# CILAB-MA/gpudrive_lab

Hardware: AMD Instinct MI355X
Metric: agent-steps/sec at 1024 worlds x 64 agents; achieved HBM GB/s on obs kernel (higher is better)
Workload: dtype f32

## Files before the change

### gpudrive_lab_amd/csrc/engine.cpp

```cpp
#include <hip/hip_runtime.h>

#include <algorithm>
#include <cmath>
#include <cstdlib>
#include <cstdio>
#include <cstring>
#include <map>
#include <memory>
#include <stdexcept>
#include <atomic>
#include <exception>
#include <string>
#include <thread>
#include <vector>

#include "dev_mem.hpp"
#include "engine.hpp"
#include "gd_math.hpp"
#include "scene.hpp"
#ifdef GD_CLOCKS
namespace gd { void set_clocks_read(unsigned long long *out); void step_clocks_read(unsigned long long *out); }
#endif
#ifndef GD_GRID_MIN_CELL
#define GD_GRID_MIN_CELL 16.f
// ... 155 lines not shown
    int64_t host_skipped = 0;
    bool rk_possible = false;
    bool rk_alloc = false;

    bool ensure_rank_buffers() {
        if (rk_alloc) return true;
        const size_t WA = static_cast<size_t>(W) * A;
        std::vector<gd::DevMem> mine;
        gd::DevSim n = d;
        try {
            alloc_into(mine, n.rk_E, WA * GD_RANK_CAP + 64);
            alloc_into(mine, n.rk_spc, WA * GD_RANK_SPL);
            if (std::getenv("GPUDRIVE_RANK_ALLOC_FAIL") != nullptr)
                throw HipError("GPUDRIVE_RANK_ALLOC_FAIL: simulated allocation failure of the rank replay's buffers");
            alloc_into(mine, n.rk_kt, WA * GD_RANK_KT);
            alloc_into(mine, n.rk_heap, WA * GD_RANK_HEAP_DW);
            alloc_into(mine, n.rk_cpe, WA * GD_RANK_NCP);
            alloc_into(mine, n.rk_n, WA);
            alloc_into(mine, n.rk_fallback, WA / 32);
            alloc_into(mine, n.rk_streak, WA / 32);
            alloc_into(mine, n.cp_road, 2 * WA * GD_RANK_NCP);
            alloc_into(mine, n.cp_T, 2 * WA * GD_RANK_NCP);
            alloc_into(mine, n.cp_hdr, 2 * WA);
            alloc_into(mine, n.rk_cp, WA * GD_RANK_NCP);
            alloc_into(mine, n.rk_tl, WA);
            alloc_into(mine, n.rk_hist, GD_RH_ALLOC);
            alloc_into(mine, n.rk_ticket, WA);
            alloc_into(mine, n.rk_order, WA);
            alloc_into(mine, n.rk_list, 8 * WA);
            n.rk_nlong = static_cast<int>(std::max<size_t>(WA / 4, 64));
            alloc_into(mine, n.rk_longlist, n.rk_nlong);
            alloc_into(mine, n.rk_longslot, WA);
            alloc_into(mine, n.rk_E_long, static_cast<size_t>(n.rk_nlong) * GD_RANK_CAP_LONG + 64);
            alloc_into(mine, n.rk_kt_long, static_cast<size_t>(n.rk_nlong) * GD_RANK_KT_LONG);
            internal.reserve(internal.size() + mine.size());
        } catch (const HipError &) {
            (void)hipGetLastError();
            rk_possible = false;
            d.rk_on = 0;
            return false;
        }
        for (gd::DevMem &m : mine) internal.push_back(std::move(m));
        d = n;
        rk_alloc = true;
        return true;
    }
    bool timing = false;
    std::vector<EventPair> ev_pool[gd::KERNEL_TIMED];
// ... 798 lines not shown
        s->lin_cap = (static_cast<size_t>(W) + 64) * static_cast<size_t>(A) + 8 * 4 * static_cast<size_t>(d.lin_apw) + 64;
        s->d_lin_list = s->alloc_internal<int32_t>(s->lin_cap);
        s->d_lin_list_dyn = s->alloc_internal<int32_t>(s->lin_cap);
        d.lin_list = s->d_lin_list; d.lin_list_dyn = s->d_lin_list_dyn;
        d.lin_blocks = 0; d.lin_blocks_dyn = 0; d.lin_dyn_off = 0;
        d.lin_on = std::getenv("GPUDRIVE_LINEAR_LEGACY") == nullptr ? 1 : 0;
        d.pose_stamp = s->alloc_internal<uint4>(WA);
        d.pose_skip = std::getenv("GPUDRIVE_NO_POSE_SKIP") == nullptr ? 1 : 0;
        d.stat_skipped = s->alloc_internal<unsigned long long>(GD_SKIP_SLOTS);
        s->d_row_of_slot = s->alloc_internal<int32_t>(WA);
        s->d_slot_of_row = s->alloc_internal<int32_t>(WA);
        s->d_row_count = s->alloc_internal<int32_t>(1);
        d.bad_actions = s->alloc_internal<unsigned long long>(1);
        d.blk_off = s->d_blk_off = s->alloc_internal<int32_t>(W + 1);
        d.warm_k = 0;
        d.warm_all = 0;
        d.warm_flags = s->alloc_internal<int32_t>(W);
        d.warm_count = s->alloc_internal<unsigned long long>(1);
        d.rk_on = 0;
        d.rk_dbg = 0;
        d.rk_min_roads = 1536;
        d.rk_waves = 0;
        if (const char *e = std::getenv("GPUDRIVE_RANK_WAVES")) d.rk_waves = std::min(std::max((std::atoi(e) + 7) / 8 * 8, 8), GD_RANK_GRID);
        s->rk_possible = GD_MAP_OBS_AW == 32 && cfg->knn_order != GD_KNN_SET_ORDER &&
                         params->roadObservationAlgorithm == GD_ROADS_K_NEAREST && std::getenv("GPUDRIVE_NO_RANK_REPLAY") == nullptr;
#ifdef GD_DIAG
        if (const char *e = std::getenv("GPUDRIVE_RANK_DBG")) d.rk_dbg = std::atoi(e);
#endif
        for (int i = 0; i < gd_sim::kRing; i++) {
            void *pinned = nullptr;
            HIP_CHECK(hipHostMalloc(&pinned, sizeof(int32_t) * W, hipHostMallocDefault));
            s->h_flags[i].reset(static_cast<int32_t *>(pinned));
            s->flag_ev[i] = make_event(hipEventDisableTiming);
        }
        std::vector<int> all(W);
        for (int w = 0; w < W; w++) all[w] = w;
        s->rebuild_worlds(all);
        s->do_reset(std::vector<int32_t>(W, 1));
        HIP_CHECK(hipStreamSynchronize(s->stream));
    });
    if (rc != GD_OK) return rc;
    *out = s.release();
    return GD_OK;
}

void gd_destroy(gd_sim *sim) { delete sim; }
// ... 1259 lines not shown
            return fail(GD_ERR_DEVICE, "gd_stat: reading the LiDAR flags failed");
        int64_t c = 0;
        for (int w = 0; w < s->W; w++)
            for (int a = 0; a < n[static_cast<size_t>(w) * 2] && a < s->A; a++) c += f[static_cast<size_t>(w) * s->A + a] != 0;
        *out = c;
        return GD_OK;
    }
    if (s && out && which == 45) {
        unsigned long long v = 0;
        (void)hipStreamSynchronize(s->stream);
        if (hipMemcpy(&v, s->d.bad_actions, sizeof(v), hipMemcpyDeviceToHost) != hipSuccess)
            return fail(GD_ERR_DEVICE, "gd_stat: reading the action counter failed");
        *out = static_cast<int64_t>(v);
        return GD_OK;
    }
    if (s && out && which == 46) {
        unsigned long long v = 0;
        (void)hipStreamSynchronize(s->stream);
        if (hipMemcpy(&v, s->d.warm_count, sizeof(v), hipMemcpyDeviceToHost) != hipSuccess)
            return fail(GD_ERR_DEVICE, "gd_stat: reading the warm-up counter failed");
        *out = static_cast<int64_t>(v);
        return GD_OK;
    }
    if (s && out && which == 21) {
        *out = 0;
        if (s->rk_alloc) {
            int32_t v = 0;
            (void)hipStreamSynchronize(s->stream);
            if (hipMemcpy(&v, s->d.rk_hist + GD_RANK_AUDIT, sizeof(v), hipMemcpyDeviceToHost) != hipSuccess)
                return fail(GD_ERR_DEVICE, "gd_stat: reading the audit counter failed");
            *out = v;
        }
        return GD_OK;
    }
    if (!s || !out || which < 0 || which > kLastStat) return fail(GD_ERR_INVALID, "gd_stat: bad argument");
#if defined(GD_DIAG) || defined(GD_CLOCKS)
    if (which >= 8) {
        *out = 0;
        if (s->rk_alloc) {
            int32_t v = 0;
            (void)hipStreamSynchronize(s->stream);
            (void)hipMemcpy(&v, s->d.rk_hist + 514 + (which - 8), sizeof(v), hipMemcpyDeviceToHost);
            (void)hipMemset(s->d.rk_hist + 514 + (which - 8), 0, sizeof(v));
            *out = v;
        }
        return GD_OK;
// ... 157 lines not shown
```

### gpudrive_lab_amd/csrc/engine.hpp

```cpp
#pragma once
#include <hip/hip_runtime.h>

#include <cstdint>

#include "../../include/gpudrive_amd.h"

#ifndef GD_MAP_OBS_AW
#define GD_MAP_OBS_AW 32
#endif

#define GD_RANK_CAP 1280
#define GD_RANK_NCP 40
#define GD_RANK_HEAP_DW 104
#define GD_RANK_CAP_LONG 2560
#define GD_RANK_KT_LONG 164
#define GD_RH_LONG 537
#define GD_RH_CURSOR 544
#define GD_RH_CURSOR_STRIDE 32
#define GD_RH_SIZE (GD_RH_CURSOR + 8 * GD_RH_CURSOR_STRIDE)
#define GD_RANK_GRID (256 * 8 * 4)
#ifdef GD_CLOCKS
#define GD_WAVE_CLOCKS
#endif
#ifdef GD_WAVE_CLOCKS
#define GD_RH_WAVES GD_RH_SIZE
#define GD_RH_ALLOC (GD_RH_WAVES + 3 * GD_RANK_GRID)
#else
#define GD_RH_ALLOC GD_RH_SIZE
#endif
#define GD_RANK_NCH 320
#define GD_RANK_SPL 256
#define GD_RANK_KT 84
#define GD_RANK_AUDIT 536
#define GD_LIN_BLK 16
#define GD_SKIP_SLOTS 4096

#ifdef GD_DIAG
#define GD_DIAG_IS(field, value) ((field) == (value))
#else
#define GD_DIAG_IS(field, value) false
#endif

namespace gd {

enum { KERNEL_STATE = 0, KERNEL_MAP_OBS = 1, KERNEL_LIDAR = 2, KERNEL_BEV = 3, KERNEL_PARTNER = 4, KERNEL_RESET = 5, KERNEL_PADDING = 6, KERNEL_TIMED = 5 };

struct GridHdr {
    float ox, oy, inv_cell;
    int nx, ny;
    int cell_base;
    int item_base;
    int pad;
// ... 65 lines not shown
    unsigned long long *bad_actions;
    unsigned long long *stat_skipped;
    int split_partner;
    int step_dbg;
    int rk_on;
    int rk_max_roads;
    int rk_min_roads;
    int rk_dbg;
    uint16_t *rk_E;
    int rk_nlong;
    int32_t *rk_longlist;
    int32_t *rk_longslot;
    uint16_t *rk_E_long;
    float *rk_kt_long;
    uint16_t *rk_spc;
    float *rk_kt;
    uint32_t *rk_heap;
    uint16_t *rk_cpe;
    int32_t *rk_hist;
    int rk_waves;
    int32_t *rk_ticket;
    int32_t *rk_order;
    int32_t *rk_list;
    uint2 *rk_cp;
    float *rk_tl;
    const float4 *road_bbox;
    const float *road_rbmax;
    int32_t *rk_n;
    int32_t *rk_fallback;
    int32_t *rk_streak;
    uint16_t *cp_road;
    float *cp_T;
    float4 *cp_hdr;
    int warm_k;
    int warm_all;
    int32_t *warm_flags;
    unsigned long long *warm_count;
    const float *pack_weights;
};

void launch_kernel(const DevSim &d, hipStream_t st, int which, bool move);
void launch_map_obs(const DevSim &d, hipStream_t st, bool move);
void launch_map_obs_rank(const DevSim &d, hipStream_t st);
void launch_map_obs_linear(const DevSim &d, hipStream_t st, bool move);
void launch_bev(const DevSim &d, hipStream_t st);
void launch_lidar(const DevSim &d, hipStream_t st);
void launch_pack_obs(const DevSim &d, hipStream_t st, float *out);
void launch_expert_actions(const DevSim &d, hipStream_t st, float *actions, float *pos, float *vel, float *yaw, int *valid);
void launch_set_log_actions(const DevSim &d, hipStream_t st, int t);
void launch_episode_step(const DevSim &d, hipStream_t st, const gd_episode_config &c, const gd_episode_buffers &b);
void launch_draw_weights(const DevSim &d, hipStream_t st, const gd_episode_config &c, const gd_episode_buffers &b,
                         const int32_t *worlds, int n);
void launch_pack_obs_rows(const DevSim &d, hipStream_t st, float *out,
                          const float *weights);
void launch_learner_rows(hipStream_t st, const uint8_t *mask, size_t slots, int32_t *row_of_slot, int32_t *slot_of_row,
                         int32_t *count);
void launch_discrete_actions(const DevSim &d, hipStream_t st, const int64_t *indices, const float *table, int n_actions);
void launch_pack_obs_conditioned(const DevSim &d, hipStream_t st, const float *weights, float *out);
void launch_record(const DevSim &d, hipStream_t st, const gd_record_buffers &b, int t, bool pre);
void launch_bc_rollout_row(const DevSim &d, hipStream_t st, const gd_bc_rollout_buffers &b, int t, int num_stack);
void launch_bc_rollout_actions(const DevSim &d, hipStream_t st, const gd_bc_rollout_buffers &b, int t);
void launch_bc_rollout_post(const DevSim &d, hipStream_t st, const gd_bc_rollout_buffers &b, int t, bool more);
void launch_bc_rollout_summary(hipStream_t st, const gd_bc_rollout_buffers &b);
void launch_policy_rollout_actions(const DevSim &d, hipStream_t st, const gd_policy_rollout_buffers &b, int t);
void launch_policy_rollout_book(const DevSim &d, hipStream_t st, const gd_policy_rollout_buffers &b, int t);
void launch_policy_rollout_finish(const DevSim &d, hipStream_t st, const gd_policy_rollout_buffers &b, int n_steps);
// ... 69 lines not shown
```

### gpudrive_lab_amd/csrc/map_obs_rank.hip

```cpp
#include <hip/hip_runtime.h>

#include <algorithm>
#include <type_traits>

#include "engine.hpp"
#include "gd_math.hpp"
#include "rank_cand.hpp"
#include "rank_heap.hpp"

namespace gd {

namespace {

constexpr int K = GD_MAP_OBS_K;
constexpr int CAP = GD_RANK_CAP;
constexpr int NCP = GD_RANK_NCP;
constexpr int SPL = GD_RANK_SPL;
constexpr int KT = GD_RANK_KT;
constexpr int TILE = 32;
constexpr int CAP_LONG = GD_RANK_CAP_LONG;
template <int CAP_T>
struct RankGeo {
    static constexpr bool LONG = CAP_T > CAP;
    static constexpr int NG = CAP_T / 64;
// ... 77 lines not shown
}
__device__ __forceinline__ uint2 stream_load(const uint2 *p) {
    const u2v v = __builtin_nontemporal_load(reinterpret_cast<const u2v *>(p));
    return make_uint2(v.x, v.y);
}
__device__ __forceinline__ void stream_store(uint2 v, uint2 *p) {
    u2v t; t.x = v.x; t.y = v.y;
    __builtin_nontemporal_store(t, reinterpret_cast<u2v *>(p));
}

__device__ __forceinline__ int audited(const DevSim &d, int idx, int size) {
    if ((unsigned int)idx < (unsigned int)size) return idx;
    atomicAdd(&d.rk_hist[GD_RANK_AUDIT], 1);
    return idx < 0 ? 0 : size - 1;
}

__device__ __forceinline__ bool rank_lt(unsigned int a, unsigned int b, unsigned int tm = 31u) { return (a | tm) < b; }

template <int A_T>
__global__ __launch_bounds__(256) void k_knn_scan(DevSim d) {
    if (d.gate_any && *d.any_reset == 0) return;
    constexpr int HALVES = A_T / 64;
    const int w = blockIdx.x / HALVES, a0 = (blockIdx.x % HALVES) * 64;
    const int tid = threadIdx.x, wave = tid >> 6, lane = tid & 63;
    const int n = d.shape[w * 2 + 0];
    if (a0 >= n) return;
    const int a = a0 + lane;
    const bool live = a < n;
    const size_t i = (size_t)w * A_T + a;
    const size_t WA = (size_t)d.W * A_T;
    const int r0 = d.road_off[w];
    const int R = d.road_off[w + 1] - r0;

    __shared__ unsigned short s_first[NCP][64];
    __shared__ float s_thr[NCP][64];
    __shared__ int s_ncp[64];
    __shared__ unsigned int s_needy[2];
    __shared__ float4 s_hdr[64];
    __shared__ float s_bx[64], s_by[64], s_bm[64];
    __shared__ unsigned int s_hist[4][256];

    float ex = 0.f, ey = 0.f;
    if (live) { ex = d.px[i]; ey = d.py[i]; }
    unsigned long long ranked = 0ull;
    int list_base = 0;
    if (wave == 0) {
        int ncp = 0;
        float4 h0 = make_float4(0.f, 0.f, __int_as_float(0), 0.f), h1 = h0;
        if (live) { h0 = d.cp_hdr[i]; h1 = d.cp_hdr[WA + i]; }
        s_hdr[lane] = h0;
        wave_sync();
        if (live) {
            const float4 bb = d.road_bbox[w];
            const float ddx = fmaxf(fmaxf(bb.x - ex, ex - bb.z), 0.f), ddy = fmaxf(fmaxf(bb.y - ey, ey - bb.w), 0.f);
            const float far = d.p.observationRadius * 1.01f + 1.f;
            int state = 1, reason = -1;
            if (R >= K && ddx * ddx + ddy * ddy > far * far) {
                state = RK_FAR;
                d.sel_hdr[i * 2] = make_float4(ex, ey, d.qw[i], d.qz[i]);
                d.sel_hdr[i * 2 + 1] = make_float4(__int_as_float(0), __int_as_float(r0), 0.f, 0.f);
                d.cp_hdr[i] = make_float4(ex, ey, __int_as_float(0), 0.f);
            } else {
                const int n0 = __float_as_int(h0.z), n1 = __float_as_int(h1.z);
                const float m0 = n0 > 0 ? sqrtf((ex - h0.x) * (ex - h0.x) + (ey - h0.y) * (ey - h0.y)) : __builtin_inff();
                const float m1 = n1 > 0 ? sqrtf((ex - h1.x) * (ex - h1.x) + (ey - h1.y) * (ey - h1.y)) : __builtin_inff();
                int set = m1 < m0 ? 1 : 0;
                float move = set ? m1 : m0;
                int n_cp = set ? n1 : n0;
                size_t src = i;
                if (move > 6.f) {
                    float best = move;
                    int donor = -1;
                    for (int j = 0; j < 64; j++) {
                        const float4 hj = s_hdr[j];
                        const float dj = __float_as_int(hj.z) > 0 ? sqrtf((ex - hj.x) * (ex - hj.x) + (ey - hj.y) * (ey - hj.y)) : __builtin_inff();
                        if (dj < best) { best = dj; donor = j; }
                    }
                    if (donor >= 0) {
                        move = best;
                        set = 0;
                        n_cp = __float_as_int(s_hdr[donor].z);
                        src = (size_t)w * A_T + a0 + donor;
                    }
                }
                const bool eligible = R >= K && R >= d.rk_min_roads && R <= d.rk_max_roads;
                const int grp = (int)(i / 32);
                const bool bypass = eligible && d.rk_streak[grp] >= 3 && ((d.rk_hist[513] + grp) & 63) != 0;
                const float iw = d.qw[i], iz = d.qz[i];
                const float z2 = iz * iz;
                const float det = (1.f - 2.f * z2) * (1.f - 2.f * z2) + 4.f * z2 * (iw * iw);
                const float margin = 1.00001f / fminf(det, 1.f);
                if (!eligible || bypass) {
                    state = 0;
                    ncp = 0;
                    reason = bypass ? -5 : -2;
                    d.rk_fallback[i / 32] = 1;
                } else if (n_cp <= 0 || move > 6.f) {
                    ncp = -1;
                    s_bx[lane] = ex; s_by[lane] = ey; s_bm[lane] = margin;
                } else {
                    ncp = n_cp;
                    const unsigned short *cr = d.cp_road + ((size_t)set * WA + src) * NCP;
                    const float *ct = d.cp_T + ((size_t)set * WA + src) * NCP;
                    float t = 1.f;
                    unsigned int fmax = 0u;
                    for (int q = 0; q < ncp; q++) {
                        t = ct[q];
                        const float reach = sqrtf(t) * 1.0001f + move * 1.0001f + 1e-3f;
                        float thr = reach * reach * 1.0001f * margin;
                        if (!(thr >= 0.f)) thr = __builtin_inff();
                        fmax = rank_cand::running_max(fmax, cr[q]);
                        s_first[q][lane] = (unsigned short)fmax;
                        s_thr[q][lane] = thr;
                    }
                    d.rk_tl[i] = t;
                }
            }
            d.rk_n[i] = state;
            d.rk_ticket[i] = reason;
            if (state == RK_FAR) ncp = 0;
        }
        s_ncp[lane] = ncp;
        {
            const unsigned long long nd = __ballot(ncp < 0);
            if (lane == 0) { s_needy[0] = (unsigned int)nd; s_needy[1] = (unsigned int)(nd >> 32); }
        }
        if (ncp < 0) ncp = 1;
        ranked = __ballot(ncp > 0);
        if (ranked != 0ull && lane == 0) list_base = atomicAdd(&d.rk_hist[528 + (blockIdx.x & 7)], __popcll(ranked));
    }
    __syncthreads();
    {
        const unsigned long long needy = (unsigned long long)s_needy[0] | (unsigned long long)s_needy[1] << 32;
        if (needy != 0ull) {
            constexpr int BASE = (127 - 2) << 4;
            unsigned int *hist = s_hist[wave];
            int turn = 0;
            for (unsigned long long rest = needy; rest != 0ull; rest &= rest - 1ull, turn++) {
                if ((turn & 3) != wave) continue;
                const int al = __ffsll((long long)rest) - 1;
                const float bx = s_bx[al], by = s_by[al], mg = s_bm[al];
#pragma unroll
                for (int k = 0; k < 4; k++) hist[k * 64 + lane] = 0u;
                if (lane == 0) { s_first[0][al] = (unsigned short)((K / 32) * 32); s_thr[0][al] = __builtin_inff(); }
                const float ratio = exp2f(log2f(fmaxf((float)R / 256.f, 1.f)) / (float)(NCP - 2));
                float pf = 256.f, tlast = __builtin_inff();
                int pq = 256, q = 1;
                float2 nxt = lane < R ? d.road_xy[r0 + lane] : make_float2(0.f, 0.f);
                for (int rb = 0; rb < R; rb += 64) {
                    const float2 xy = nxt;
                    if (rb + 64 + lane < R) nxt = d.road_xy[r0 + rb + 64 + lane];
                    if (rb + lane < R) {
// ... 9 lines not shown
                        int jb = 0, before = excl;
                        if (before + (int)h.x < K) { before += (int)h.x; jb = 1;
                            if (before + (int)h.y < K) { before += (int)h.y; jb = 2;
                                if (before + (int)h.z < K) { jb = 3; } } }
                        const unsigned long long cross = __ballot(excl < K && incl >= K);
                        const int Lc = __ffsll((long long)cross) - 1;
                        const int bucket = 4 * Lc + __builtin_amdgcn_readlane(jb, Lc);
                        const float T = bucket >= 255 ? __builtin_inff() : __uint_as_float((unsigned int)(bucket + 1 + BASE) << 19);
                        if (lane == 0) {
                            const float reach = sqrtf(T) * 1.0001f + 1e-3f;
                            float thr = reach * reach * 1.0001f * mg * 1.001f;
                            if (!(thr >= 0.f)) thr = __builtin_inff();
                            s_first[q][al] = (unsigned short)min(pq, 65535);
                            s_thr[q][al] = thr;
                        }
                        tlast = T;
                        q++;
                        pf *= ratio;
                        pq = max(pq + 64, ((int)pf + 63) & ~63);
                    }
                }
                if (lane == 0) {
                    s_ncp[al] = q;
                    d.rk_tl[(size_t)w * A_T + a0 + al] = tlast < 1e30f ? tlast : 1.f;
                }
            }
            __syncthreads();
        }
    }
    const int ncp = s_ncp[lane];
    if (__syncthreads_or(ncp > 0 ? 1 : 0) == 0) return;
    {
        uint2 *rows = d.rk_cp + ((size_t)w * A_T + a0) * NCP;
        for (int e = tid; e < 64 * NCP; e += 256) {
            const int ag = e / NCP, q = e - ag * NCP;
            const int n_ag = s_ncp[ag];
            if (n_ag > 0)
                rows[e] = q < n_ag ? make_uint2((unsigned int)s_first[q][ag], __float_as_uint(s_thr[q][ag]))
                                   : make_uint2(rank_cand::NO_CP, __float_as_uint(__builtin_inff()));
        }
    }
    if (wave == 0 && ranked != 0ull) {
        list_base = __builtin_amdgcn_readfirstlane(list_base);
        if (ncp > 0)
            d.rk_list[(size_t)(blockIdx.x & 7) * WA + audited(d, list_base + __popcll(ranked & ((1ull << lane) - 1ull)), (int)WA)] = (int)i;
    }
}

template <int CAP_T>
struct RankLds {
    union {
        struct {
            float ckey[CAP_T];
            unsigned short cidx[CAP_T];
        } c;
        struct {
            float skey[CAP_T];
            unsigned short spos[CAP_T];
        } s;
        unsigned short spc[CAP_T];
    };
    unsigned int cnt2[RankGeo<CAP_T>::NB / 2];
};
static_assert(sizeof(RankLds<CAP>) <= 10240 && sizeof(RankLds<CAP_LONG>) <= 20480, "sixteen / eight waves per CU");
constexpr int LSTN = (GD_MAX_ROAD_ENTITIES + GD_LIN_BLK - 1) / GD_LIN_BLK + 15;
constexpr int LSTN4 = (LSTN + 3) & ~3;
static_assert(LSTN4 <= 1024 && NCP < 64 && rank_cand::CHUNK % GD_LIN_BLK == 0 && 64 % GD_LIN_BLK == 0, "block and count share 16 bits; a block inside one chunk; whole blocks per pass");
constexpr size_t CAND_TABLES = LSTN4 * sizeof(unsigned short) + (NCP + 1) * sizeof(float);
static_assert(CAND_TABLES <= sizeof(RankLds<CAP>::cnt2) && CAND_TABLES <= sizeof(RankLds<CAP_LONG>::cnt2), "the tables fit the idle counters of both instantiations");
constexpr int CP_EPL = ((GD_MAX_ROAD_ENTITIES + rank_cand::CHUNK - 1) / rank_cand::CHUNK + 63) / 64;
static_assert(64 * CP_EPL * (sizeof(unsigned int) + sizeof(uint2)) <= sizeof(float) * CAP, "the chunk table fits the candidate keys of both instantiations");

struct RankIn {
    int i, state, r0, R, b0, li;
    float ex, ey, iw, iz, t_last;
    unsigned int cfirst;
    float cthr;
};
template <typename T>
__device__ __forceinline__ T uniform_load(const T *p) {
    return *reinterpret_cast<const __attribute__((address_space(4))) T *>(reinterpret_cast<uintptr_t>(p));
}
template <int A_T>
__device__ __forceinline__ RankIn rank_fetch(const DevSim &d, const int *list, int li, int count, int lane) {
    RankIn in;
    in.li = li;
    in.i = li < count ? uniform_load(list + li) : 0;
    in.state = li < count ? uniform_load(d.rk_n + in.i) : 0;
    const int w = in.i / A_T;
    in.r0 = uniform_load(d.road_off + w);
    in.R = uniform_load(d.road_off + w + 1) - in.r0;
    in.ex = uniform_load(d.px + in.i); in.ey = uniform_load(d.py + in.i);
    in.iw = uniform_load(d.qw + in.i); in.iz = -uniform_load(d.qz + in.i);
    in.t_last = uniform_load(d.rk_tl + in.i);
    in.b0 = uniform_load(d.blk_off + w);
    uint2 cp = make_uint2(rank_cand::NO_CP, __float_as_uint(__builtin_inff()));
    if (in.state == 1 && lane < NCP) cp = stream_load(d.rk_cp + (size_t)in.i * NCP + (unsigned int)lane);
    in.cfirst = cp.x;
    in.cthr = __uint_as_float(cp.y);
    return in;
}

#ifdef GD_CLOCKS
struct PhaseClock {
    unsigned int prev, sum[8];
    __device__ __forceinline__ void mark(int n) {
        const unsigned int t = (unsigned int)__builtin_amdgcn_s_memtime();
        sum[n] += t - prev;
        prev = t;
    }
};
#define GD_PHASE(n) clk.mark(n)
#else
struct PhaseClock {};
#define GD_PHASE(n)
#endif
__device__ __forceinline__ int rank_draw(int *cursor, int lane) {
    int e = 0;
    if (lane == 0) e = atomicAdd(cursor, 1);
    return e;
}
template <int A_T, int CAP_T>
__device__ __forceinline__ void rank_agent(const DevSim &d, const RankIn &in, int lane, RankLds<CAP_T> &L, PhaseClock &clk, int drawn,
                                           int count, const int *list, RankIn &nxt) {
    using G = RankGeo<CAP_T>;
    constexpr int NB = G::NB, NLIN = G::NLIN, NMAX = G::NMAX;
    constexpr unsigned int TM = (1u << G::RSH) - 1u;
    if (__builtin_amdgcn_readfirstlane(in.state) != 1) {
        nxt = rank_fetch<A_T>(d, list, __builtin_amdgcn_readfirstlane(drawn), count, lane);
        return;
    }
    auto uni = [](int v) -> int { return __builtin_amdgcn_readfirstlane(v); };
    auto unif = [](float v) -> float { return __int_as_float(__builtin_amdgcn_readfirstlane(__float_as_int(v))); };
    const int i = uni(in.i), r0 = uni(in.r0), R = uni(in.R);
    const int group = i / 32;
    constexpr int NG = G::NG;

    const float ex = unif(in.ex), ey = unif(in.ey), iw = unif(in.iw), iz = unif(in.iz);
    unsigned short *const lst = reinterpret_cast<unsigned short *>(L.cnt2);
    float *const tthr = reinterpret_cast<float *>(L.cnt2) + LSTN4 / 2;
    const unsigned int cfirst = in.cfirst;
    if (lane < NCP) tthr[lane + 1] = in.cthr;
    if (lane == 63) tthr[0] = __builtin_inff();
    const float creach = rank_cand::block_reach(in.cthr);
    const int nblk = (R + GD_LIN_BLK - 1) / GD_LIN_BLK;
    const int nch = rank_cand::chunks_of(R), epl = (nch + 63) >> 6;
    unsigned int *const tmax = reinterpret_cast<unsigned int *>(L.c.ckey);
    uint2 *const tcp = reinterpret_cast<uint2 *>(L.c.ckey + 64 * CP_EPL);
#pragma unroll
    for (int u = 0; u < CP_EPL; u++)
        if (u < epl) tmax[u * 64 + lane] = 0u;
    wave_sync();
    if (lane < NCP && rank_cand::cp_table_takes(cfirst, nch)) atomicMax(&tmax[rank_cand::cp_table_chunk(cfirst)], rank_cand::cp_table_entry(lane));
    wave_sync();
    {
        int own[CP_EPL], run = 0;
#pragma unroll
        for (int u = 0; u < CP_EPL; u++) own[u] = u < epl ? (int)tmax[lane * epl + u] : 0;
#pragma unroll
        for (int u = 0; u < CP_EPL; u++) { run = max(run, own[u]); own[u] = run; }
        const int before = __builtin_amdgcn_ds_bpermute(((lane - 1) & 63) << 2, wave_incl_max_nonneg(run));
#pragma unroll
        for (int u = 0; u < CP_EPL; u++)
            if (u < epl) {
                const int cnt = lane ? max(own[u], before) : own[u];
                const int reach = __builtin_amdgcn_ds_bpermute(((cnt - 1) & 63) << 2, __float_as_int(creach));
                tcp[lane * epl + u] = make_uint2((unsigned int)cnt, (unsigned int)reach);
// ... 139 lines not shown
                    d.rk_fallback[group] = 1;
                }
            }
            return;
        }
    }
#ifdef GD_CLOCKS
    clk.sum[7] += (unsigned int)((nsv + 3) / 4) << 8;
#endif
    const int bin = 255 - min(255, (nin - K) / 5);
    int ticket = 0;
    if (lane == 0) ticket = bin << 20 | atomicAdd(&d.rk_hist[bin], 1);
    GD_PHASE(1);
    if (GD_DIAG_IS(d.rk_dbg, 1)) return;
    if (lane <= (nin - K) >> G::TSH) {
        const int road = (int)L.c.cidx[K - 1 + (lane << G::TSH)];
        d.cp_road[(size_t)i * NCP + lane] = (unsigned short)(lane ? min(65535, (road + 1 + 31) & ~31) : (K / 32) * 32);
    }
    constexpr int GQ = 5;
    static_assert(NG % GQ == 0, "whole groups");
    const float kmax = d.radius_key_max;
    int ci[NG];
    float key[NG];
    const float t_last = unif(in.t_last);
    float split = (t_last > 0.f && t_last < 1e30f) ? t_last * 1.5f : 1.f;
    int nle = 0, nlow = 0;
    float kmax_seen = 0.f, kmin_seen = __builtin_inff();
#pragma unroll
    for (int g0 = 0; g0 < NG; g0 += GQ) {
#pragma unroll
        for (int u = 0; u < GQ; u++) { ci[g0 + u] = 0; key[g0 + u] = 0.f; }
        if (g0 * 64 < nin) {
            int v[GQ];
            float kv[GQ];
#pragma unroll
            for (int u = 0; u < GQ; u++) {
                v[u] = (int)L.c.cidx[(g0 + u) * 64 + lane];
                kv[u] = L.c.ckey[(g0 + u) * 64 + lane];
            }
            static_assert(GQ == 5, "operand list");
            asm volatile("" : "+v"(v[0]), "+v"(v[1]), "+v"(v[2]), "+v"(v[3]), "+v"(v[4]), "+v"(kv[0]), "+v"(kv[1]), "+v"(kv[2]), "+v"(kv[3]), "+v"(kv[4]));
#pragma unroll
            for (int u = 0; u < GQ; u++) {
                const int g = g0 + u;
                const bool on = g * 64 + lane < nin;
                ci[g] = on ? v[u] : 0;
                key[g] = on ? kv[u] : 0.f;
// ... 196 lines not shown
    }
    if (lane == 0) {
        d.rk_n[i] = nin | (nle << 16) | (has_tie ? 1 << 28 : 0) | (G::LONG ? 1 << 29 : 0);
        if (G::LONG) d.rk_longslot[i] = uni(in.li);
        d.rk_ticket[i] = ticket;
    }
    GD_PHASE(6);
}

template <int A_T, int CAP_T>
__global__ __launch_bounds__(64, CAP_T > CAP ? 2 : 4) void k_knn_rank(DevSim d) {
    if (d.gate_any && *d.any_reset == 0) return;
    __shared__ RankLds<CAP_T> L;
    constexpr bool LONG = RankGeo<CAP_T>::LONG;
    const int xcd = blockIdx.x & 7;
    const int count = LONG ? min(uniform_load(d.rk_hist + GD_RH_LONG), d.rk_nlong) : uniform_load(d.rk_hist + 528 + xcd);
    const int *list = LONG ? d.rk_longlist : d.rk_list + (size_t)xcd * d.W * A_T;
    int *const cursor = d.rk_hist + GD_RH_CURSOR + xcd * GD_RH_CURSOR_STRIDE;
    const int share = LONG ? (int)gridDim.x : (int)(gridDim.x >> 3), mine = LONG ? (int)blockIdx.x : (int)(blockIdx.x >> 3);
    const bool fixed = LONG || count <= share;
#ifdef GD_WAVE_CLOCKS
    int turns = 0;
    if (!LONG && threadIdx.x == 0) {
        d.rk_hist[GD_RH_WAVES + blockIdx.x] = (int)__builtin_amdgcn_s_memrealtime();
        d.rk_hist[GD_RH_WAVES + 2 * GD_RANK_GRID + blockIdx.x] = 0;
    }
#endif
    if (fixed && mine >= count) return;
    int t = fixed ? mine : __builtin_amdgcn_readfirstlane(rank_draw(cursor, threadIdx.x));
    RankIn cur = rank_fetch<A_T>(d, list, t, count, threadIdx.x);
    PhaseClock clk;
#ifdef GD_CLOCKS
    for (int k = 0; k < 8; k++) clk.sum[k] = 0u;
    clk.prev = (unsigned int)__builtin_amdgcn_s_memtime();
#endif
    while (t < count) {
        RankIn nxt;
        GD_PHASE(0);
        int lane_v = threadIdx.x;
        asm volatile("" : "+v"(lane_v));
        const int drawn = fixed ? t + share : rank_draw(cursor, lane_v);
        rank_agent<A_T, CAP_T>(d, cur, lane_v, L, clk, drawn, count, list, nxt);
        wave_sync();
        cur = nxt;
        t = __builtin_amdgcn_readfirstlane(nxt.li);
#ifdef GD_WAVE_CLOCKS
        turns++;
#endif
    }
#ifdef GD_CLOCKS
    if (threadIdx.x == 0)
// ... 34 lines not shown
    const int tl = threadIdx.x;
    const int c = d.rk_hist[tl];
    const int incl = wave_incl_scan(c);
    if ((tl & 63) == 63) s_part[tl >> 6] = incl;
    __syncthreads();
    int before = 0;
    for (int k = 0; k < (tl >> 6); k++) before += s_part[k];
    s_start[tl] = before + incl - c;
    if (blockIdx.x == 0 && tl == 255) {
        d.rk_hist[512] = before + incl;
        d.rk_hist[513]++;
        for (int x = 0; x < 8; x++) d.rk_hist[528 + x] = 0;
        d.rk_hist[GD_RH_LONG] = 0;
        for (int x = 0; x < 8; x++) d.rk_hist[GD_RH_CURSOR + x * GD_RH_CURSOR_STRIDE] = 0;
    }
#ifdef GD_CLOCKS
    if (blockIdx.x == 0) d.rk_hist[256 + tl] = 0;
#endif
    __syncthreads();
    const int t = blockIdx.x * 256 + tl;
    if (t >= d.live_count) return;
    const int i = d.live_list[t];
    const int ticket = d.rk_ticket[i];
    if (ticket < 0) return;
    d.rk_order[audited(d, s_start[(ticket >> 20) & 255] + (ticket & 0xfffff), d.W * d.A)] = i;
}

#ifdef GD_CLOCKS
struct ReplayClock {
    unsigned int prev, first, ph[5];
    __device__ __forceinline__ void start() { first = prev = (unsigned int)__builtin_amdgcn_s_memrealtime(); }
    __device__ __forceinline__ void mark(int n) {
        const unsigned int t = (unsigned int)__builtin_amdgcn_s_memrealtime();
        ph[n] = t - prev;
        prev = t;
    }
};
#define GD_RPHASE(n) rclk.mark(n)
#else
#define GD_RPHASE(n)
#endif
__global__ __launch_bounds__(64) void k_knn_replay(DevSim d) {
    if (d.gate_any && *d.any_reset == 0) return;
    const int lane = threadIdx.x;
#ifdef GD_CLOCKS
    ReplayClock rclk;
// ... 300 lines not shown
    const size_t WA = (size_t)d.W * A_T;
    if (lane < ncp) {
        (void)audited(d, cp_slot, n);
        d.cp_T[(size_t)i * NCP + lane] = cp_t;
        if (at_start) {
            d.cp_T[(WA + i) * NCP + lane] = cp_t;
            d.cp_road[(WA + i) * NCP + lane] = cp_r;
        }
    }
    if (lane == 0) {
        d.rk_streak[i / 32] = 0;
        d.cp_hdr[i] = make_float4(ex, ey, __int_as_float(ncp), 0.f);
        if (at_start) d.cp_hdr[WA + i] = make_float4(ex, ey, __int_as_float(ncp), 0.f);
        d.sel_hdr[(size_t)i * 2] = make_float4(ex, ey, qw, qz);
        d.sel_hdr[(size_t)i * 2 + 1] = make_float4(__int_as_float(m), __int_as_float(r0), __int_as_float(1), 0.f);
    }
}

}

#ifndef GD_RANK_LONG_GRID
#define GD_RANK_LONG_GRID 2048
#endif
void launch_map_obs_rank(const DevSim &d, hipStream_t st) {
    if (d.live_count == 0) return;
    const dim3 glong(std::min(std::max(d.rk_nlong, 1), GD_RANK_LONG_GRID));
    const dim3 gr(d.rk_waves > 0 ? d.rk_waves : std::min((d.live_count + 7) / 8 * 8, GD_RANK_GRID)), g4((d.live_count + 3) / 4), gw(d.W * (d.A / 64));
    if (d.A == 64) {
        hipLaunchKernelGGL((k_knn_scan<64>), gw, dim3(256), 0, st, d);
        hipLaunchKernelGGL((k_knn_rank<64, CAP>), gr, dim3(64), 0, st, d);
        if (d.rk_nlong > 0) hipLaunchKernelGGL((k_knn_rank<64, CAP_LONG>), glong, dim3(64), 0, st, d);
    } else {
        hipLaunchKernelGGL((k_knn_scan<128>), gw, dim3(256), 0, st, d);
        hipLaunchKernelGGL((k_knn_rank<128, CAP>), gr, dim3(64), 0, st, d);
        if (d.rk_nlong > 0) hipLaunchKernelGGL((k_knn_rank<128, CAP_LONG>), glong, dim3(64), 0, st, d);
    }
    hipLaunchKernelGGL(k_knn_order, dim3((d.live_count + 255) / 256), dim3(256), 0, st, d);
    hipLaunchKernelGGL(k_knn_replay, dim3((d.live_count + AWR - 1) / AWR), dim3(64), 0, st, d);
    if (d.A == 64) hipLaunchKernelGGL((k_knn_finish<64>), g4, dim3(256), 0, st, d);
    else hipLaunchKernelGGL((k_knn_finish<128>), g4, dim3(256), 0, st, d);
}

}
```

### gpudrive_lab_amd/csrc/rank_cand.hpp

```cpp
#pragma once

#include <cmath>

#if defined(__HIPCC__)
#define GD_RC_FN __host__ __device__ __forceinline__
#else
#define GD_RC_FN inline
#endif

namespace gd {
namespace rank_cand {

constexpr int CHUNK = 32;
constexpr unsigned int NO_CP = 0xffffffffu;

GD_RC_FN unsigned int f32_bits(float f) { return __builtin_bit_cast(unsigned int, f); }

GD_RC_FN bool road_passes(float x, float y, float ex, float ey, float thr) {
    const float dx = x - ex, dy = y - ey;
    const float d2 = __builtin_fmaf(dx, dx, dy * dy);
    return (f32_bits(d2 - thr) >> 31) != 0u;
}
GD_RC_FN bool is_candidate(int r, int K, int R, float x, float y, float ex, float ey, float thr) {
    return r < R && (r < K || road_passes(x, y, ex, ey, thr));
}

GD_RC_FN int cp_in_force(const unsigned int *first, int ncp, int base) {
    int q = -1;
    while (q + 1 < ncp && first[q + 1] <= (unsigned int)base) q++;
    return q;
}
GD_RC_FN unsigned int running_max(unsigned int run, unsigned int first) { return first > run ? first : run; }
GD_RC_FN int cp_count(const unsigned int *first_max, int n, int base) {
    int c = 0;
    for (int q = 0; q < n; q++) c += first_max[q] <= (unsigned int)base ? 1 : 0;
    return c;
}
GD_RC_FN int chunk_base_of_block(int b, int blk) { return (b * blk) & ~(CHUNK - 1); }

GD_RC_FN int chunks_of(int R) { return (R + CHUNK - 1) / CHUNK; }
GD_RC_FN unsigned int cp_table_chunk(unsigned int first_max) { return first_max / CHUNK + (first_max % CHUNK ? 1u : 0u); }
GD_RC_FN bool cp_table_takes(unsigned int first_max, int nchunks) {
    return first_max != NO_CP && cp_table_chunk(first_max) < (unsigned int)nchunks;
}
GD_RC_FN unsigned int cp_table_entry(int q) { return (unsigned int)q + 1u; }
GD_RC_FN void cp_table(unsigned int *tab, int nchunks, const unsigned int *first_max, int n) {
    for (int c = 0; c < nchunks; c++) tab[c] = 0u;
    for (int q = 0; q < n; q++)
        if (cp_table_takes(first_max[q], nchunks)) {
            unsigned int &e = tab[cp_table_chunk(first_max[q])];
            e = cp_table_entry(q) > e ? cp_table_entry(q) : e;
        }
    for (int c = 1; c < nchunks; c++) tab[c] = tab[c - 1] > tab[c] ? tab[c - 1] : tab[c];
}

GD_RC_FN float block_reach(float thr) { return sqrtf(thr) * 1.00001f; }
GD_RC_FN bool block_survives(int b, int blk, int K, float cx, float cy, float rad, float ex, float ey, float reach) {
    const float dx = cx - ex, dy = cy - ey, rr = reach + rad;
    return b * blk < K || !(dx * dx + dy * dy > rr * rr * 1.00001f);
}

}
// ... 2 lines not shown
```

Measured before the change: 69.46 million.

## Skip per-agent candidate row copy when agent owns its checkpoints; cap rank grid residency

When an agent's checkpoint data is its own (no donor), the scan kernel now writes only a small per-agent record, and the rank kernel reads the cp_road/cp_T arrays directly and computes thresholds and running max in-wave. The old interleaved uint2 row buffer is split into separate first/threshold arrays, and t_last moves into the record. Persistent rank blocks beyond the occupancy-derived resident count exit early, and the list index is dealt with a rotation instead of blockIdx&7. The intent is to cut global writes and reads of candidate rows and reduce redundant block launches, at the cost of extra in-kernel arithmetic and a row-counter atomic.

```diff
diff --git a/gpudrive_lab_amd/csrc/engine.cpp b/gpudrive_lab_amd/csrc/engine.cpp
--- a/gpudrive_lab_amd/csrc/engine.cpp
+++ b/gpudrive_lab_amd/csrc/engine.cpp
@@ -201,8 +201,9 @@
             alloc_into(mine, n.cp_road, 2 * WA * GD_RANK_NCP);
             alloc_into(mine, n.cp_T, 2 * WA * GD_RANK_NCP);
             alloc_into(mine, n.cp_hdr, 2 * WA);
-            alloc_into(mine, n.rk_cp, WA * GD_RANK_NCP);
-            alloc_into(mine, n.rk_tl, WA);
+            alloc_into(mine, n.rk_cpf, WA * GD_RANK_NCP);
+            alloc_into(mine, n.rk_cpt, WA * GD_RANK_NCP);
+            alloc_into(mine, n.rk_rec, WA);
             alloc_into(mine, n.rk_hist, GD_RH_ALLOC);
             alloc_into(mine, n.rk_ticket, WA);
             alloc_into(mine, n.rk_order, WA);
@@ -1047,6 +1048,9 @@
         d.rk_min_roads = 1536;
         d.rk_waves = 0;
         if (const char *e = std::getenv("GPUDRIVE_RANK_WAVES")) d.rk_waves = std::min(std::max((std::atoi(e) + 7) / 8 * 8, 8), GD_RANK_GRID);
+        d.rk_scan_rows = 0;
+        if (const char *e = std::getenv("GPUDRIVE_RANK_SCAN_ROWS")) d.rk_scan_rows = std::atoi(e) != 0 ? 1 : 0;
+        d.rk_resident = std::max(gd::rank_resident_waves(A) / 8, 1);
         s->rk_possible = GD_MAP_OBS_AW == 32 && cfg->knn_order != GD_KNN_SET_ORDER &&
                          params->roadObservationAlgorithm == GD_ROADS_K_NEAREST && std::getenv("GPUDRIVE_NO_RANK_REPLAY") == nullptr;
 #ifdef GD_DIAG
@@ -2352,6 +2356,17 @@
         *out = static_cast<int64_t>(v);
         return GD_OK;
     }
+    if (s && out && which == 22) {
+        *out = 0;
+        if (s->rk_alloc) {
+            int32_t v = 0;
+            (void)hipStreamSynchronize(s->stream);
+            if (hipMemcpy(&v, s->d.rk_hist + GD_RH_ROWS, sizeof(v), hipMemcpyDeviceToHost) != hipSuccess)
+                return fail(GD_ERR_DEVICE, "gd_stat: reading the row counter failed");
+            *out = v;
+        }
+        return GD_OK;
+    }
     if (s && out && which == 21) {
         *out = 0;
         if (s->rk_alloc) {
diff --git a/gpudrive_lab_amd/csrc/engine.hpp b/gpudrive_lab_amd/csrc/engine.hpp
--- a/gpudrive_lab_amd/csrc/engine.hpp
+++ b/gpudrive_lab_amd/csrc/engine.hpp
@@ -15,6 +15,7 @@
 #define GD_RANK_CAP_LONG 2560
 #define GD_RANK_KT_LONG 164
 #define GD_RH_LONG 537
+#define GD_RH_ROWS 538
 #define GD_RH_CURSOR 544
 #define GD_RH_CURSOR_STRIDE 32
 #define GD_RH_SIZE (GD_RH_CURSOR + 8 * GD_RH_CURSOR_STRIDE)
@@ -28,6 +29,7 @@
 #else
 #define GD_RH_ALLOC GD_RH_SIZE
 #endif
+#define GD_RK_REC_ROW (1 << 16)
 #define GD_RANK_NCH 320
 #define GD_RANK_SPL 256
 #define GD_RANK_KT 84
@@ -139,8 +141,11 @@
     int32_t *rk_ticket;
     int32_t *rk_order;
     int32_t *rk_list;
-    uint2 *rk_cp;
-    float *rk_tl;
+    uint16_t *rk_cpf;
+    float *rk_cpt;
+    float4 *rk_rec;
+    int rk_scan_rows;
+    int rk_resident;
     const float4 *road_bbox;
     const float *road_rbmax;
     int32_t *rk_n;
@@ -159,6 +164,7 @@
 void launch_kernel(const DevSim &d, hipStream_t st, int which, bool move);
 void launch_map_obs(const DevSim &d, hipStream_t st, bool move);
 void launch_map_obs_rank(const DevSim &d, hipStream_t st);
+int rank_resident_waves(int A);
 void launch_map_obs_linear(const DevSim &d, hipStream_t st, bool move);
 void launch_bev(const DevSim &d, hipStream_t st);
 void launch_lidar(const DevSim &d, hipStream_t st);
diff --git a/gpudrive_lab_amd/csrc/map_obs_rank.hip b/gpudrive_lab_amd/csrc/map_obs_rank.hip
--- a/gpudrive_lab_amd/csrc/map_obs_rank.hip
+++ b/gpudrive_lab_amd/csrc/map_obs_rank.hip
@@ -123,6 +123,8 @@
     if (d.gate_any && *d.any_reset == 0) return;
     constexpr int HALVES = A_T / 64;
     const int w = blockIdx.x / HALVES, a0 = (blockIdx.x % HALVES) * 64;
+    const int xl = d.rk_scan_rows ? (int)(blockIdx.x & 7) : rank_cand::deal_list((int)blockIdx.x, (int)gridDim.x);
+    if (blockIdx.x == 0 && threadIdx.x == 0) d.rk_hist[GD_RH_ROWS] = 0;
     const int tid = threadIdx.x, wave = tid >> 6, lane = tid & 63;
     const int n = d.shape[w * 2 + 0];
     if (a0 >= n) return;
@@ -144,6 +146,8 @@
     float ex = 0.f, ey = 0.f;
     if (live) { ex = d.px[i]; ey = d.py[i]; }
     unsigned long long ranked = 0ull;
+    bool own_cp = false;
+    bool listed = false;
     int list_base = 0;
     if (wave == 0) {
         int ncp = 0;
@@ -169,7 +173,7 @@
                 float move = set ? m1 : m0;
                 int n_cp = set ? n1 : n0;
                 size_t src = i;
-                if (move > 6.f) {
+                if (move > rank_cand::CP_MOVE_MAX) {
                     float best = move;
                     int donor = -1;
                     for (int j = 0; j < 64; j++) {
@@ -196,39 +200,41 @@
                     ncp = 0;
                     reason = bypass ? -5 : -2;
                     d.rk_fallback[i / 32] = 1;
-                } else if (n_cp <= 0 || move > 6.f) {
+                } else if (n_cp <= 0 || move > rank_cand::CP_MOVE_MAX) {
                     ncp = -1;
                     s_bx[lane] = ex; s_by[lane] = ey; s_bm[lane] = margin;
+                } else if (src == i && !d.rk_scan_rows) {
+                    ncp = n_cp;
+                    own_cp = true;
+                    d.rk_rec[i] = make_float4(move, margin, __int_as_float(n_cp | set << 8), 0.f);
                 } else {
                     ncp = n_cp;
+                    float t = 1.f;
                     const unsigned short *cr = d.cp_road + ((size_t)set * WA + src) * NCP;
                     const float *ct = d.cp_T + ((size_t)set * WA + src) * NCP;
-                    float t = 1.f;
                     unsigned int fmax = 0u;
                     for (int q = 0; q < ncp; q++) {
                         t = ct[q];
-                        const float reach = sqrtf(t) * 1.0001f + move * 1.0001f + 1e-3f;
-                        float thr = reach * reach * 1.0001f * margin;
-                        if (!(thr >= 0.f)) thr = __builtin_inff();
                         fmax = rank_cand::running_max(fmax, cr[q]);
                         s_first[q][lane] = (unsigned short)fmax;
-                        s_thr[q][lane] = thr;
+                        s_thr[q][lane] = rank_cand::cp_threshold(t, move, margin);
                     }
-                    d.rk_tl[i] = t;
+                    d.rk_rec[i] = make_float4(move, t, __int_as_float(n_cp | GD_RK_REC_ROW), 0.f);
                 }
             }
             d.rk_n[i] = state;
             d.rk_ticket[i] = reason;
             if (state == RK_FAR) ncp = 0;
         }
-        s_ncp[lane] = ncp;
+        s_ncp[lane] = own_cp ? 0 : ncp;
         {
             const unsigned long long nd = __ballot(ncp < 0);
             if (lane == 0) { s_needy[0] = (unsigned int)nd; s_needy[1] = (unsigned int)(nd >> 32); }
         }
         if (ncp < 0) ncp = 1;
         ranked = __ballot(ncp > 0);
-        if (ranked != 0ull && lane == 0) list_base = atomicAdd(&d.rk_hist[528 + (blockIdx.x & 7)], __popcll(ranked));
+        listed = ncp > 0;
+        if (ranked != 0ull && lane == 0) list_base = atomicAdd(&d.rk_hist[528 + xl], __popcll(ranked));
     }
     __syncthreads();
     {
@@ -284,28 +290,29 @@
                 }
                 if (lane == 0) {
                     s_ncp[al] = q;
-                    d.rk_tl[(size_t)w * A_T + a0 + al] = tlast < 1e30f ? tlast : 1.f;
+                    d.rk_rec[(size_t)w * A_T + a0 + al] = make_float4(0.f, tlast < 1e30f ? tlast : 1.f, __int_as_float(q | GD_RK_REC_ROW), 0.f);
                 }
             }
             __syncthreads();
         }
+    }
+    if (wave == 0 && ranked != 0ull) {
+        list_base = __builtin_amdgcn_readfirstlane(list_base);
+        if (listed)
+            d.rk_list[(size_t)xl * WA + audited(d, list_base + __popcll(ranked & ((1ull << lane) - 1ull)), (int)WA)] = (int)i;
     }
     const int ncp = s_ncp[lane];
     if (__syncthreads_or(ncp > 0 ? 1 : 0) == 0) return;
     {
-        uint2 *rows = d.rk_cp + ((size_t)w * A_T + a0) * NCP;
+        unsigned short *rowf = d.rk_cpf + ((size_t)w * A_T + a0) * NCP;
+        float *rowt = d.rk_cpt + ((size_t)w * A_T + a0) * NCP;
         for (int e = tid; e < 64 * NCP; e += 256) {
             const int ag = e / NCP, q = e - ag * NCP;
-            const int n_ag = s_ncp[ag];
-            if (n_ag > 0)
-                rows[e] = q < n_ag ? make_uint2((unsigned int)s_first[q][ag], __float_as_uint(s_thr[q][ag]))
-                                   : make_uint2(rank_cand::NO_CP, __float_as_uint(__builtin_inff()));
-        }
-    }
-    if (wave == 0 && ranked != 0ull) {
-        list_base = __builtin_amdgcn_readfirstlane(list_base);
-        if (ncp > 0)
-            d.rk_list[(size_t)(blockIdx.x & 7) * WA + audited(d, list_base + __popcll(ranked & ((1ull << lane) - 1ull)), (int)WA)] = (int)i;
+            if (q < s_ncp[ag]) {
+                rowf[e] = s_first[q][ag];
+                rowt[e] = s_thr[q][ag];
+            }
+        }
     }
 }
 
@@ -328,16 +335,18 @@
 constexpr int LSTN = (GD_MAX_ROAD_ENTITIES + GD_LIN_BLK - 1) / GD_LIN_BLK + 15;
 constexpr int LSTN4 = (LSTN + 3) & ~3;
 static_assert(LSTN4 <= 1024 && NCP < 64 && rank_cand::CHUNK % GD_LIN_BLK == 0 && 64 % GD_LIN_BLK == 0, "block and count share 16 bits; a block inside one chunk; whole blocks per pass");
-constexpr size_t CAND_TABLES = LSTN4 * sizeof(unsigned short) + (NCP + 1) * sizeof(float);
+constexpr size_t CAND_TABLES = LSTN4 * sizeof(unsigned short) + (NCP + 2) * sizeof(float);
 static_assert(CAND_TABLES <= sizeof(RankLds<CAP>::cnt2) && CAND_TABLES <= sizeof(RankLds<CAP_LONG>::cnt2), "the tables fit the idle counters of both instantiations");
 constexpr int CP_EPL = ((GD_MAX_ROAD_ENTITIES + rank_cand::CHUNK - 1) / rank_cand::CHUNK + 63) / 64;
 static_assert(64 * CP_EPL * (sizeof(unsigned int) + sizeof(uint2)) <= sizeof(float) * CAP, "the chunk table fits the candidate keys of both instantiations");
 
 struct RankIn {
     int i, state, r0, R, b0, li;
-    float ex, ey, iw, iz, t_last;
+    float ex, ey, iw, iz;
     unsigned int cfirst;
     float cthr;
+    float rec_move, rec_y;
+    int rec_pack;
 };
 template <typename T>
 __device__ __forceinline__ T uniform_load(const T *p) {
@@ -354,12 +363,19 @@
     in.R = uniform_load(d.road_off + w + 1) - in.r0;
     in.ex = uniform_load(d.px + in.i); in.ey = uniform_load(d.py + in.i);
     in.iw = uniform_load(d.qw + in.i); in.iz = -uniform_load(d.qz + in.i);
-    in.t_last = uniform_load(d.rk_tl + in.i);
     in.b0 = uniform_load(d.blk_off + w);
-    uint2 cp = make_uint2(rank_cand::NO_CP, __float_as_uint(__builtin_inff()));
-    if (in.state == 1 && lane < NCP) cp = stream_load(d.rk_cp + (size_t)in.i * NCP + (unsigned int)lane);
-    in.cfirst = cp.x;
-    in.cthr = __uint_as_float(cp.y);
+    const float *rec = reinterpret_cast<const float *>(d.rk_rec + in.i);
+    in.rec_move = uniform_load(rec); in.rec_y = uniform_load(rec + 1); in.rec_pack = __float_as_int(uniform_load(rec + 2));
+    const bool has_row = (in.rec_pack & GD_RK_REC_ROW) != 0;
+    const size_t own = ((size_t)((in.rec_pack >> 8) & 1) * d.W * A_T + in.i) * NCP, row = (size_t)in.i * NCP;
+    const unsigned short *pf = has_row ? d.rk_cpf + row : d.cp_road + own;
+    const float *pt = has_row ? d.rk_cpt + row : d.cp_T + own;
+    in.cfirst = rank_cand::NO_CP;
+    in.cthr = __builtin_inff();
+    if (in.state == 1 && lane < min(in.rec_pack & 0xff, NCP)) {
+        in.cfirst = pf[(unsigned int)lane];
+        in.cthr = pt[(unsigned int)lane];
+    }
     return in;
 }
 
@@ -401,10 +417,19 @@
     const float ex = unif(in.ex), ey = unif(in.ey), iw = unif(in.iw), iz = unif(in.iz);
     unsigned short *const lst = reinterpret_cast<unsigned short *>(L.cnt2);
     float *const tthr = reinterpret_cast<float *>(L.cnt2) + LSTN4 / 2;
-    const unsigned int cfirst = in.cfirst;
-    if (lane < NCP) tthr[lane + 1] = in.cthr;
+    unsigned int cfirst = in.cfirst;
+    float cthr = in.cthr, t_last_in = unif(in.rec_y);
+    if (!(uni(in.rec_pack) & GD_RK_REC_ROW)) {
+        const int n_own = min(uni(in.rec_pack) & 0xff, NCP);
+        const bool have = lane < n_own;
+        t_last_in = __int_as_float(__builtin_amdgcn_readlane(__float_as_int(cthr), n_own - 1));
+        const unsigned int fmax = (unsigned int)wave_incl_max_nonneg(have ? (int)cfirst : 0);
+        cthr = have ? rank_cand::cp_threshold(cthr, unif(in.rec_move), unif(in.rec_y)) : __builtin_inff();
+        cfirst = have ? fmax : rank_cand::NO_CP;
+    }
+    if (lane <= NCP) tthr[lane + 1] = lane < NCP ? cthr : t_last_in;
     if (lane == 63) tthr[0] = __builtin_inff();
-    const float creach = rank_cand::block_reach(in.cthr);
+    const float creach = rank_cand::block_reach(cthr);
     const int nblk = (R + GD_LIN_BLK - 1) / GD_LIN_BLK;
     const int nch = rank_cand::chunks_of(R), epl = (nch + 63) >> 6;
     unsigned int *const tmax = reinterpret_cast<unsigned int *>(L.c.ckey);
@@ -590,7 +615,7 @@
     const float kmax = d.radius_key_max;
     int ci[NG];
     float key[NG];
-    const float t_last = unif(in.t_last);
+    const float t_last = unif(tthr[NCP + 1]);
     float split = (t_last > 0.f && t_last < 1e30f) ? t_last * 1.5f : 1.f;
     int nle = 0, nlow = 0;
     float kmax_seen = 0.f, kmin_seen = __builtin_inff();
@@ -833,11 +858,14 @@
 #ifdef GD_WAVE_CLOCKS
     int turns = 0;
     if (!LONG && threadIdx.x == 0) {
-        d.rk_hist[GD_RH_WAVES + blockIdx.x] = (int)__builtin_amdgcn_s_memrealtime();
+        const int now = (int)__builtin_amdgcn_s_memrealtime();
+        d.rk_hist[GD_RH_WAVES + blockIdx.x] = now;
+        d.rk_hist[GD_RH_WAVES + GD_RANK_GRID + blockIdx.x] = now;
         d.rk_hist[GD_RH_WAVES + 2 * GD_RANK_GRID + blockIdx.x] = 0;
     }
 #endif
     if (fixed && mine >= count) return;
+    if (!fixed && mine >= d.rk_resident) return;
     int t = fixed ? mine : __builtin_amdgcn_readfirstlane(rank_draw(cursor, threadIdx.x));
     RankIn cur = rank_fetch<A_T>(d, list, t, count, threadIdx.x);
     PhaseClock clk;
@@ -918,6 +946,10 @@
     if (t >= d.live_count) return;
     const int i = d.live_list[t];
     const int ticket = d.rk_ticket[i];
+    {
+        const unsigned long long rows = __ballot(ticket >= 0 && (__float_as_int(d.rk_rec[i].z) & GD_RK_REC_ROW) != 0);
+        if (rows != 0ull && (tl & 63) == 0) atomicAdd(&d.rk_hist[GD_RH_ROWS], __popcll(rows));
+    }
     if (ticket < 0) return;
     d.rk_order[audited(d, s_start[(ticket >> 20) & 255] + (ticket & 0xfffff), d.W * d.A)] = i;
 }
@@ -1264,6 +1296,18 @@
 #ifndef GD_RANK_LONG_GRID
 #define GD_RANK_LONG_GRID 2048
 #endif
+int rank_resident_waves(int A) {
+    int per_cu = 0, dev = 0;
+    hipDeviceProp_t prop;
+    const hipError_t e = A == 64 ? hipOccupancyMaxActiveBlocksPerMultiprocessor(&per_cu, k_knn_rank<64, CAP>, 64, 0)
+                                 : hipOccupancyMaxActiveBlocksPerMultiprocessor(&per_cu, k_knn_rank<128, CAP>, 64, 0);
+    if (e != hipSuccess || hipGetDevice(&dev) != hipSuccess || hipGetDeviceProperties(&prop, dev) != hipSuccess) {
+        (void)hipGetLastError();
+        return GD_RANK_GRID;
+    }
+    return std::max(per_cu, 1) * std::max(prop.multiProcessorCount, 1);
+}
+
 void launch_map_obs_rank(const DevSim &d, hipStream_t st) {
     if (d.live_count == 0) return;
     const dim3 glong(std::min(std::max(d.rk_nlong, 1), GD_RANK_LONG_GRID));
diff --git a/gpudrive_lab_amd/csrc/rank_cand.hpp b/gpudrive_lab_amd/csrc/rank_cand.hpp
--- a/gpudrive_lab_amd/csrc/rank_cand.hpp
+++ b/gpudrive_lab_amd/csrc/rank_cand.hpp
@@ -38,6 +38,23 @@
 }
 GD_RC_FN int chunk_base_of_block(int b, int blk) { return (b * blk) & ~(CHUNK - 1); }
 
+GD_RC_FN float cp_threshold(float t, float move, float margin) {
+    const float reach = sqrtf(t) * 1.0001f + move * 1.0001f + 1e-3f;
+    const float thr = reach * reach * 1.0001f * margin;
+    return thr >= 0.f ? thr : __builtin_inff();
+}
+constexpr float CP_MOVE_MAX = 6.f;
+
+GD_RC_FN int deal_rotation(int g) { return (g + (g >> 3) + (g >> 6)) & 7; }
+GD_RC_FN int deal_block(int b, int grid) {
+    if ((b | 7) >= grid) return b;
+    return (b & ~7) | ((b + deal_rotation(b >> 3)) & 7);
+}
+GD_RC_FN int deal_list(int w, int grid) {
+    if ((w | 7) >= grid) return w & 7;
+    return (w - deal_rotation(w >> 3)) & 7;
+}
+
 GD_RC_FN int chunks_of(int R) { return (R + CHUNK - 1) / CHUNK; }
 GD_RC_FN unsigned int cp_table_chunk(unsigned int first_max) { return first_max / CHUNK + (first_max % CHUNK ? 1u : 0u); }
 GD_RC_FN bool cp_table_takes(unsigned int first_max, int nchunks) {
```

Result: faster. 70.52 million, median of 6 (+1.5%).
